# NREL/SSRS

Measured on AMD Instinct MI355X. Metric: simulated tracks/sec (whole node), higher is better.
Workload: dtype f64

## Files before the change

ssrs_amd/csrc/tracks.hip:

```cpp
#include <rocrand/rocrand_philox4x32_10.h>
#include <hipcub/hipcub.hpp>

#include <cmath>
#include <cstdlib>
#include <cstring>
#include <new>
#include <vector>

#include "common.h"
#include "track_plan.h"
#include "track_policy.h"

namespace ssrs {

__host__ __device__ constexpr int dr_of(int k) { return k / 3 - 1; }
__host__ __device__ constexpr int dc_of(int k) { return k % 3 - 1; }
#define SSRS_NINV_DIAG 0.70710677f

constexpr uint32_t restriction(int d)
{
    const int dr = dr_of(d), dc = dc_of(d);
    uint32_t m = 0;
    for (int k = 0; k < 9; ++k) {
        bool ok = false;
// ... 55 lines not shown
    for (int c = 0; c < 8; ++c)
        if (kRingK[c] == k) return c;
    return 8;
}
constexpr bool ring_matches_restrictions()
{
    for (int c = 0; c < 8; ++c) {
        const uint32_t m = (1u << kRingK[(c + 7) % 8]) | (1u << kRingK[c]) | (1u << kRingK[(c + 1) % 8]);
        if (m != restriction(kRingK[c])) return false;
    }
    return true;
}
static_assert(ring_matches_restrictions(), "restriction(d) = ring neighbours of d");
constexpr uint32_t ring_order(int c)
{
    const int ks[3] = {kRingK[(c + 7) % 8], kRingK[c], kRingK[(c + 1) % 8]};
    uint32_t v = 0;
    int n = 0;
    for (int k = 0; k < 9; ++k)
        for (int j = 0; j < 3; ++j)
            if (ks[j] == k) v |= static_cast<uint32_t>(j) << (2 * n++);
    return v;
}
constexpr uint64_t pack_ring_orders()
{
    uint64_t v = 0;
    for (int c = 0; c < 8; ++c) v |= static_cast<uint64_t>(ring_order(c)) << (6 * c);
    return v;
}
constexpr uint64_t kRingOrder = pack_ring_orders();
constexpr uint32_t kOrdId = 0u | (1u << 2) | (2u << 4), kOrdRot = 2u | (0u << 2) | (1u << 4),
                   kOrdRev = 2u | (1u << 2) | (0u << 4), kOrdSwp = 1u | (0u << 2) | (2u << 4);
static_assert(ring_order(0) == kOrdId && ring_order(6) == kOrdId && ring_order(7) == kOrdId, "x0 x1 x2");
static_assert(ring_order(1) == kOrdRot, "after NE: x2 x0 x1");
static_assert(ring_order(2) == kOrdRev && ring_order(3) == kOrdRev && ring_order(4) == kOrdRev, "x2 x1 x0");
static_assert(ring_order(5) == kOrdSwp, "after SW: x1 x0 x2");
static_assert(ring_order(0) == (0u | (1u << 2) | (2u << 4)), "after N: NW, N, NE are k = 6, 7, 8");
static_assert(ring_order(2) == (2u | (1u << 2) | (0u << 4)), "after E: NE, E, SE are k = 8, 5, 2");
constexpr uint32_t pack_ring_deltas(bool rows)
{
    uint32_t v = 1u << 16;
    for (int c = 0; c < 8; ++c)
        v |= static_cast<uint32_t>((rows ? dr_of(kRingK[c]) : dc_of(kRingK[c])) + 1) << (2 * c);
    return v;
}
constexpr uint32_t kRingDr = pack_ring_deltas(true), kRingDc = pack_ring_deltas(false);
constexpr uint32_t pack_ring_next(int sel)
{
    uint32_t v = 0;
    for (int c = 0; c < 8; ++c) v |= static_cast<uint32_t>((c + 7 + ((ring_order(c) >> (2 * sel)) & 3u)) & 7u) << (4 * c);
    return v;
}
constexpr uint32_t kRingNext0 = pack_ring_next(0), kRingNext1 = pack_ring_next(1), kRingNext2 = pack_ring_next(2);
constexpr uint32_t pack_ring_deltas_signed(bool rows)
{
    uint32_t v = 0;
    for (int c = 0; c < 8; ++c)
        v |= (static_cast<uint32_t>(rows ? dr_of(kRingK[c]) : dc_of(kRingK[c])) & 3u) << (4 * c);
    return v;
}
constexpr uint32_t kRingDrS = pack_ring_deltas_signed(true), kRingDcS = pack_ring_deltas_signed(false);
constexpr uint64_t pack_ring_of_k()
{
    uint64_t v = 0;
    for (int k = 0; k < 9; ++k) v |= static_cast<uint64_t>(ring_of_k(k)) << (4 * k);
    return v;
}
constexpr uint64_t kRingOfK = pack_ring_of_k();
constexpr uint64_t pack_k_of_ring()
{
    uint64_t v = 4ull << 32;
    for (int c = 0; c < 8; ++c) v |= static_cast<uint64_t>(kRingK[c]) << (4 * c);
    return v;
}
constexpr uint64_t kKOfRing = pack_k_of_ring();
constexpr int kRingFloats = 10;
__host__ __device__ constexpr size_t ring_mask_offset(int rows, int cols)
{
    return static_cast<size_t>(rows) * static_cast<size_t>(cols) * kRingFloats * sizeof(float) + 8;
}

__device__ __forceinline__ uint4 philox_block(uint64_t seed, uint64_t track, uint64_t blk)
{
#ifdef SSRS_PROBE_NO_PHILOX
    const uint32_t h = static_cast<uint32_t>(blk) * 0x9E3779B9u ^ static_cast<uint32_t>(track) * 0x85EBCA6Bu ^
                       static_cast<uint32_t>(seed);
    return make_uint4(h * 0xC2B2AE35u, h ^ 0x27D4EB2Fu, (h >> 3) * 0x165667B1u, h + 0x9E3779B9u);
#endif
    rocrand_state_philox4x32_10 st;
    rocrand_init(seed, track, blk * 4ull, &st);
    return rocrand4(&st);
}

__device__ __forceinline__ uint4 philox_block_b3(uint64_t seed, uint64_t track, uint64_t blk)
{
    uint32_t c0 = static_cast<uint32_t>(blk), c1 = static_cast<uint32_t>(blk >> 32);
    uint32_t c2 = static_cast<uint32_t>(track), c3 = static_cast<uint32_t>(track >> 32);
    uint32_t k0 = static_cast<uint32_t>(seed), k1 = static_cast<uint32_t>(seed >> 32);
#pragma unroll
    for (int r = 0; r < 10; ++r) {
        const uint64_t p0 = static_cast<uint64_t>(0xD2511F53u) * c0, p1 = static_cast<uint64_t>(0xCD9E8D57u) * c2;
        const uint32_t n0 = __builtin_amdgcn_bitop3_b32(static_cast<uint32_t>(p1 >> 32), c1, k0, 0x96);
        const uint32_t n2 = __builtin_amdgcn_bitop3_b32(static_cast<uint32_t>(p0 >> 32), c3, k1, 0x96);
        c1 = static_cast<uint32_t>(p1);
        c3 = static_cast<uint32_t>(p0);
        c0 = n0;
// ... 1537 lines not shown
    }
    const unsigned long long live = __ballot(active);
    const int lane = threadIdx.x & 63;
    const int nsurv = __popcll(live);
    uint32_t basei = 0;
    if (HM == 6) {
        __shared__ uint32_t s_surv[kBlock / 64 + 1];
        const int wv = threadIdx.x >> 6;
        if (lane == 0) s_surv[wv] = static_cast<uint32_t>(nsurv);
        __syncthreads();
        if (threadIdx.x == 0) {
            uint32_t tot = 0;
            for (int q = 0; q < kBlock / 64; ++q) tot += s_surv[q];
            s_surv[kBlock / 64] = tot ? atomicAdd(&ctl->count[out_slot][xcd], static_cast<uint32_t>(kBlock)) : 0xFFFFFFFFu;
        }
        __syncthreads();
        basei = s_surv[kBlock / 64];
        if (basei != 0xFFFFFFFFu) {
            a.list_out[xcd * a.cap + basei + threadIdx.x] = active ? t : -1;
            if (active) {
                TrackState o;
                o.pos = static_cast<int32_t>(row | (col << 16));
                o.k = k;
                o.dirs = static_cast<uint32_t>(kKOfRing >> (4 * rc)) & 0xFu;
                o.aux = s.aux;
                a.state[t] = o;
            }
        }
    } else {
        if (lane == 0 && nsurv) basei = atomicAdd(&ctl->count[out_slot][xcd], static_cast<uint32_t>(nsurv));
        basei = __shfl(basei, 0);
    }
    if (HM != 6 && active) {
        const int rank = __popcll(live & ((1ull << lane) - 1ull));
        a.list_out[xcd * a.cap + basei + rank] = t;
        TrackState o;
        o.pos = static_cast<int32_t>(row | (col << 16));
        o.k = k;
        o.dirs = static_cast<uint32_t>(kKOfRing >> (4 * rc)) & 0xFu;
        o.aux = s.aux;
        a.state[t] = o;
    }
    unsigned long long mv = live0 ? static_cast<unsigned long long>(k - s.k) : 0ull;
#pragma unroll
    for (int off = 32; off > 0; off >>= 1) mv += __shfl_down(mv, off);
    if (lane == 0 && mv) atomicAdd(&ctl->steps, mv);
}

struct alignas(16) RoamEntry {
    uint32_t e0, ea, eb, ec;
};
static_assert(sizeof(RoamEntry) == 16, "one dwordx4 per state");
constexpr size_t kPairMaxCells = 1ull << 25;

template <bool REV>
__global__ __launch_bounds__(kBlock) void k_roam_build(const char *__restrict__ tab, uint32_t guard, int plane_shift,
                                                      int rows, int cols, RoamEntry *__restrict__ out, const ThrPrior pr)
{
    const uint32_t nstate = static_cast<uint32_t>(rows) * static_cast<uint32_t>(cols) * 8u;
    for (uint32_t s = blockIdx.x * kBlock + threadIdx.x; s < nstate; s += gridDim.x * kBlock) {
        const uint32_t rc = s & 7u, cell = s >> 3;
        auto entry = [&](uint32_t c, uint32_t q) {
            return *reinterpret_cast<const uint32_t *>(tab + (guard + (q << plane_shift)) + (c << 2));
        };
        uint4 en = make_uint4(entry(cell, rc), kThrPoison, kThrPoison, kThrPoison);
        const bool rev = REV && en.x == kThrReversal;
        const uint32_t eu = rev ? pr.rev_e : en.x, rcd = rev ? pr.rev_rc : rc;
        if ((eu & 0xFFFFu) <= (eu >> 16)) {
            const uint32_t ord = static_cast<uint32_t>(kRingOrder >> (6u * rcd)) & 63u;
            uint32_t es[3];
#pragma unroll
            for (int j = 0; j < 3; ++j) {
                const uint32_t ncj = (rcd + 7u + ((ord >> (2 * j)) & 3u)) & 7u;
                const uint32_t cj = cell + ((kRingDr >> (2u * ncj)) & 3u) * static_cast<uint32_t>(cols) + ((kRingDc >> (2u * ncj)) & 3u) -
                                    static_cast<uint32_t>(cols) - 1u;
                es[j] = entry(cj, ncj);
            }
            en.y = es[0]; en.z = es[1]; en.w = es[2];
        }
        reinterpret_cast<uint4 *>(out)[s] = en;
    }
}

struct FineEntry { uint32_t t1, t2; };
struct FinePrior { uint32_t zero_t1[8], zero_t2[8], reversal; };

__host__ __device__ __forceinline__ uint32_t fine_fixed(double x)
{
    const double v = x * 4294967296.0 + 0.5;
    return v >= 4294967295.0 ? 0xFFFFFFFFu : static_cast<uint32_t>(static_cast<unsigned long long>(v));
}

template <bool HAS_POT>
__global__ __launch_bounds__(kBlock) void k_fine_build(const double *__restrict__ updraft, const float *__restrict__ potential,
                                                      FineEntry *__restrict__ out, int rows, int cols, int tiles_x, int ntiles,
                                                      const FinePrior fp)
{
    constexpr int LW = kTabW + 2, LH = kTabH + 2;
    __shared__ double s_inv[LW * LH];
    __shared__ float s_pot[LW * LH];
    const int t = xcd_band(blockIdx.x, ntiles);
    const int r0 = (t / tiles_x) * kTabH, c0 = (t % tiles_x) * kTabW;
    for (int i = threadIdx.x; i < LW * LH; i += kBlock) {
        const int lr = i / LW, lc = i - lr * LW;
        int gr = r0 - 1 + lr, gc = c0 - 1 + lc;
        gr = gr < 0 ? 0 : (gr >= rows ? rows - 1 : gr);
        gc = gc < 0 ? 0 : (gc >= cols ? cols - 1 : gc);
        const size_t g = static_cast<size_t>(gr) * cols + gc;
        const double v = updraft[g];
        const double w = v != v ? v : (v > 1e-06 ? v : 1e-06);
        s_inv[i] = 1.0 / w;
        s_pot[i] = HAS_POT ? potential[g] : 0.f;
    }
    __syncthreads();
    const int lc = static_cast<int>(threadIdx.x % kTabW) + 1;
    const int col = c0 + lc - 1;
    if (col >= cols) return;
    for (int lr = static_cast<int>(threadIdx.x / kTabW) + 1; lr <= kTabH; lr += kBlock / kTabW) {
        const int row = r0 + lr - 1;
        if (row >= rows) break;
        const size_t cell = static_cast<size_t>(row) * cols + col;
        const bool interior = row > 0 && col > 0 && row < rows - 1 && col < cols - 1;
        double w[9];
        bool bad = !interior;
        if (interior) {
            const double ic = s_inv[lr * LW + lc];
            const float pc = s_pot[lr * LW + lc];
#pragma unroll
            for (int j = 0; j < 9; ++j) {
                const int o = (lr + dr_of(j)) * LW + lc + dc_of(j);
                w[j] = 2.0 / (ic + s_inv[o]);
                if (HAS_POT) {
                    const float d = pc - s_pot[o];
                    const float ninv = (j == 4) ? 0.f : ((j & 1) ? 1.f : SSRS_NINV_DIAG);
                    const float e = d * ninv;
                    w[j] = w[j] * static_cast<double>(e);
                }
                bad |= !(w[j] - w[j] == 0.0);
                w[j] = w[j] > 0.0 ? w[j] : 0.0;
            }
        }
        FineEntry en[8];
#pragma unroll
        for (int rc = 0; rc < 8; ++rc) {
            const uint32_t ord = ring_order(rc);
            const int ring3[3] = {(rc + 7) % 8, rc, (rc + 1) % 8};
            const int ka = kRingK[ring3[ord & 3u]], kb = kRingK[ring3[(ord >> 2) & 3u]], kc = kRingK[ring3[(ord >> 4) & 3u]];
            FineEntry e = {0xFFFFFFFFu, 0u};
            if (!bad) {
                const double ab = w[ka] + w[kb], tot = ab + w[kc];
                if (tot == 0.0) {
                    if (!((fp.reversal >> rc) & 1u)) { e.t1 = fp.zero_t1[rc]; e.t2 = fp.zero_t2[rc]; }
                } else if (tot - tot == 0.0) {
                    e.t1 = fine_fixed(w[ka] / tot);
                    e.t2 = fine_fixed(ab / tot);
                    if (e.t1 > e.t2) e.t1 = e.t2;
                }
            }
            en[rc] = e;
        }
        uint4 *dst = reinterpret_cast<uint4 *>(out + cell * 8);
#pragma unroll
        for (int q = 0; q < 4; ++q) dst[q] = make_uint4(en[2 * q].t1, en[2 * q].t2, en[2 * q + 1].t1, en[2 * q + 1].t2);
    }
}

template <bool REV, int BT = kBlock>
__global__ __launch_bounds__(BT) void k_step_roam(const StepArgs a, const ThrPrior pr)
{
    __shared__ uint32_t s_win[kWinRows * kWinCols];
    __shared__ int s_box[4];
    __shared__ int s_wid[BT / 64];
    for (int q = threadIdx.x; q < kWinRows * kWinCols; q += BT) s_win[q] = 0u;
    if (threadIdx.x == 0) { s_box[0] = s_box[1] = 0x7fffffff; s_box[2] = s_box[3] = -1; }
    __syncthreads();
    TrackCtl *ctl = a.ctl;
    const int in_slot = a.launch & 3, out_slot = (a.launch + 1) & 3;
    const uint32_t xcd = blockIdx.x % kXcd;
    const uint32_t nlive = ctl->count[in_slot][xcd];
    const uint32_t il = (blockIdx.x / kXcd) * BT + threadIdx.x;
    const uint32_t i = xcd * a.cap + il;
    if (blockIdx.x == 0 && threadIdx.x < kXcd) ctl->count[(a.launch + 2) & 3][threadIdx.x] = 0;

    bool live0 = il < nlive;
    int32_t t = live0 ? (a.list_in ? a.list_in[i] : static_cast<int32_t>(i)) : 0;
    if (t < 0) { live0 = false; t = 0; }
    TrackState s = {0, -1, 0, 0};
    if (live0) s = a.state[t];
    uint32_t rc = static_cast<uint32_t>(kRingOfK >> (4 * (s.dirs & 0xFu))) & 0xFu;
    live0 = live0 && s.k >= 0 && rc < 8u;
    rc &= 7u;
    int row = s.pos & 0xFFFF, col = (s.pos >> 16) & 0xFFFF;
    int win_r0 = 0, win_c0 = 0;
    {
        int r_lo = live0 ? row : 0x7fffffff, r_hi = live0 ? row : -1, c_lo = live0 ? col : 0x7fffffff, c_hi = live0 ? col : -1;
#pragma unroll
        for (int off = 32; off > 0; off >>= 1) {
            int o = __shfl_xor(r_lo, off); r_lo = o < r_lo ? o : r_lo;
            o = __shfl_xor(r_hi, off); r_hi = o > r_hi ? o : r_hi;
            o = __shfl_xor(c_lo, off); c_lo = o < c_lo ? o : c_lo;
            o = __shfl_xor(c_hi, off); c_hi = o > c_hi ? o : c_hi;
        }
        if ((threadIdx.x & 63) == 0 && r_hi >= 0) {
            atomicMin(&s_box[0], r_lo); atomicMin(&s_box[1], c_lo);
            atomicMax(&s_box[2], r_hi); atomicMax(&s_box[3], c_hi);
        }
        __syncthreads();
        const bool fits = s_box[2] - s_box[0] < kWinRows && s_box[3] - s_box[1] < kWinCols;
        const int nwin = a.wander->n;
        int wid = live0 && nwin > 0 ? wander_window_of(a.wander, nwin, row, col) : 0x7fffffff;
        wid = wid >= nwin ? 0x7fffffff : wid;
        {
            const unsigned long long lm = __ballot(wid != 0x7fffffff);
            wid = lm ? __shfl(wid, __ffsll(static_cast<long long>(lm)) - 1) : 0x7fffffff;
        }
        if ((threadIdx.x & 63) == 0) s_wid[threadIdx.x >> 6] = wid;
        __syncthreads();
        wid = 0x7fffffff;
        for (int q = BT / 64 - 1; q >= 0; --q) wid = s_wid[q] != 0x7fffffff ? s_wid[q] : wid;
        if (wid != 0x7fffffff && threadIdx.x == 0) {
            s_box[0] = a.wander->r0[wid]; s_box[2] = s_box[0] + kWinRows - 1;
            s_box[1] = a.wander->c0[wid]; s_box[3] = s_box[1] + kWinCols - 1;
        }
        const bool placed = wid != 0x7fffffff;
        __syncthreads();
        if (!placed && !fits && threadIdx.x == 0) { s_box[0] = r_lo; s_box[1] = c_lo; s_box[2] = r_hi; s_box[3] = c_hi; }
        __syncthreads();
        if (s_box[2] >= 0) {
            win_r0 = (s_box[0] + s_box[2] + 1 - kWinRows) / 2;
            win_c0 = (s_box[1] + s_box[3] + 1 - kWinCols) / 2;
        }
    }
    const char *pair = reinterpret_cast<const char *>(a.roam);
    const uint32_t ucols = static_cast<uint32_t>(a.cols);
    const uint32_t last_cell = static_cast<uint32_t>(a.rows) * ucols - 1u;
    int k = s.k;
    const long long rel64 = (a.coherent ? static_cast<long long>(s.aux >> 9) : 0) + 1 - a.it_base;
    const int rel = rel64 > 0x3fffffffLL ? 0x3fffffff : (rel64 < 0 ? 0 : static_cast<int>(rel64));
    const long long left = a.max_k - k;
    uint32_t span = !live0 ? 0u : (left > 0x3fffffffLL ? 0x3fffffffu : (left < 0 ? 0u : static_cast<uint32_t>(left)));
    const int blk0 = (k - rel) >> 1;
    const unsigned long long track = a.track_base + static_cast<unsigned long long>(t);
    const char *tab = reinterpret_cast<const char *>(a.table);
    const uint32_t psh = static_cast<uint32_t>(a.plane_shift);
    const uint32_t rev_e = pr.rev_e;
    uint32_t win_stray = 0, n_fine = 0;
    const void *fine = a.fine;

    int wr = 0, wc = 0, lcell = 0;
    bool fast = false;
    uint4 E = make_uint4(kThrPoison, kThrPoison, kThrPoison, kThrPoison);
    auto enter = [&](bool released) __attribute__((always_inline)) {
        wr = row - win_r0;
        wc = col - win_c0;
        lcell = row * a.cols + col;
        fast = live0 && released && span != 0u && k > a.burnin;
        const uint32_t sidx = fast ? ((static_cast<uint32_t>(lcell) << 3) | rc) : 0u;
        E = *reinterpret_cast<const uint4 *>(pair + (sidx << 4));
    };
    enter(rel == 0);
    const uint32_t rev_rc4 = 4u * pr.rev_rc;

    auto slow_step = [&](const uint32_t w0, const uint32_t w1) __attribute__((always_inline)) {
        const uint32_t ufi = w0 >> 16;
        const uint32_t cell = static_cast<uint32_t>(row) * ucols + static_cast<uint32_t>(col);
        const uint32_t e = *reinterpret_cast<const uint32_t *>(tab + (a.guard + (rc << psh)) + (cell << 2));
        const int32_t d1 = static_cast<int32_t>(ufi) - static_cast<int32_t>(e & 0xFFFFu);
        const int32_t d2 = static_cast<int32_t>(ufi) - static_cast<int32_t>(e >> 16);
        const bool burn = k <= a.burnin;
        bool special = (static_cast<uint32_t>(d1 + 1) < 2u) | (static_cast<uint32_t>(d2 + 1) < 2u) | (d1 < d2);
        if (burn) special |= (row <= 1) | (row >= a.rows - 2) | (col >= a.cols - 2);
        uint32_t nc;
        int br = row, bc = col;
        if (!special) {
            const uint32_t ord = static_cast<uint32_t>(kRingOrder >> (6u * rc)) & 63u;
            const uint32_t neg = (static_cast<uint32_t>(d1) >> 31) + (static_cast<uint32_t>(d2) >> 31);
            nc = (rc + 7u + ((ord >> (4u - 2u * neg)) & 3u)) & 7u;
        } else {
            if (e == kThrBoundary && !burn) { span = 0u; return; }
            bool exact = true;
            nc = 0;
            if (fine && !(d1 < d2) && !(burn && ((row <= 1) | (row >= a.rows - 2) | (col >= a.cols - 2)))) {
                const uint2 f = reinterpret_cast<const uint2 *>(fine)[(cell << 3) | rc];
                const uint32_t u32 = (w0 & ~31u) | (w1 >> 27);
                const long long f1 = static_cast<long long>(u32) - static_cast<long long>(f.x);
                const long long f2 = static_cast<long long>(u32) - static_cast<long long>(f.y);
                const bool unsure = (f.x > f.y) | (static_cast<unsigned long long>(f1 + 1) < 2ull) | (static_cast<unsigned long long>(f2 + 1) < 2ull);
                if (!unsure) {
                    const uint32_t ord = static_cast<uint32_t>(kRingOrder >> (6u * rc)) & 63u;
                    const uint32_t neg = (f1 < 0 ? 1u : 0u) + (f2 < 0 ? 1u : 0u);
                    nc = (rc + 7u + ((ord >> (4u - 2u * neg)) & 3u)) & 7u;
                    exact = false;
                    ++n_fine;
                }
            }
            if (e == kThrReversal && !burn) {
                int idx = 0;
                bool near = false;
#pragma unroll
                for (int q = 0; q < 9; ++q) {
                    const int32_t d = static_cast<int32_t>(ufi) - static_cast<int32_t>(pr.thr9[q]);
                    idx += d >= 0 ? 1 : 0;
                    near |= static_cast<uint32_t>(d + 1) < 2u;
                }
                const uint32_t pnc = static_cast<uint32_t>(kRingOfK >> (4 * (idx > 8 ? 4 : idx))) & 0xFu;
                if (!near && pnc < 8u) { nc = pnc; exact = false; }
            }
            if (exact) {
                int er = row, ec = col;
                if (burn) {
                    if (er <= 1) er += 2; else if (er >= a.rows - 2) er -= 2;
                    if (ec <= 0) ec += 2; else if (ec >= a.cols - 2) ec -= 2;
                }
                double w[9];
                if (a.potential) window_weights<true>(a.updraft, a.potential, a.cols, er, ec, w);
                else window_weights<false>(a.updraft, a.potential, a.cols, er, ec, w);
                double prr[9];
#pragma unroll
                for (int j = 0; j < 9; ++j) prr[j] = a.prior[j];
                const uint32_t last = static_cast<uint32_t>(kKOfRing >> (4 * rc)) & 0xFu;
                const int idx = choose_move(w, prr, 1.0, restriction_of(last), words_to_uniform(w0, w1), true);
                nc = static_cast<uint32_t>(kRingOfK >> (4 * idx)) & 0xFu;
                br = er; bc = ec;
            }
        }
        row = br + static_cast<int>((kRingDr >> (2u * nc)) & 3u) - 1;
        col = bc + static_cast<int>((kRingDc >> (2u * nc)) & 3u) - 1;
        rc = nc;
        ++k;
        const uint32_t hr = static_cast<uint32_t>(row - win_r0), hc = static_cast<uint32_t>(col - win_c0);
        if (hr < static_cast<uint32_t>(kWinRows) && hc < static_cast<uint32_t>(kWinCols)) {
            atomicAdd(&s_win[hr * kWinCols + hc], 1u);
        } else {
            atomicAdd(&a.hist[static_cast<uint32_t>(row) * ucols + static_cast<uint32_t>(col)], 1u);
            ++win_stray;
        }
    };

    int it = 0;
    uint32_t n_pairs = 0, n_slow = 0;
    const unsigned long long t_begin = a.debug_roam ? __builtin_amdgcn_s_memtime() : 0ull;
    auto one_pair = [&]() __attribute__((always_inline)) {
        const uint4 w4 = philox_block_b3(a.seed, track, static_cast<unsigned long long>(static_cast<uint32_t>(blk0 + (it >> 1))));
        const uint32_t ufa = w4.x >> 16, ufb = w4.z >> 16;
        const bool st_a = static_cast<uint32_t>(it - rel) < span, st_b = static_cast<uint32_t>(it + 1 - rel) < span;
        const uint32_t q0 = E.x, qa = E.y, qb = E.z, qc = E.w;
        const uint32_t rc0 = rc;
        const uint32_t rc04 = 4u * rc0;
        const bool rva = REV && q0 == kThrReversal;
        const uint32_t eua = rva ? rev_e : q0;
        const uint32_t t4a = rva ? rev_rc4 : rc04;
        const bool ga1 = ufa >= (eua & 0xFFFFu), ga2 = ufa >= (eua >> 16);
        const uint32_t nxa = ga2 ? kRingNext2 : (ga1 ? kRingNext1 : kRingNext0);
        const uint32_t nca = (nxa >> t4a) & 7u, nca4 = 4u * nca;
        const uint32_t q1 = ga2 ? qc : (ga1 ? qb : qa);
        const int dra = __builtin_amdgcn_sbfe(static_cast<int>(kRingDrS), nca4, 2u), dca = __builtin_amdgcn_sbfe(static_cast<int>(kRingDcS), nca4, 2u);
        const int cell_a = lcell + __mul24(dra, a.cols) + dca;
        const bool rvb = REV && q1 == kThrReversal;
        const uint32_t eub = rvb ? rev_e : q1;
        const uint32_t t4b = rvb ? rev_rc4 : nca4;
        const bool gb1 = ufb >= (eub & 0xFFFFu), gb2 = ufb >= (eub >> 16);
        const uint32_t nxb = gb2 ? kRingNext2 : (gb1 ? kRingNext1 : kRingNext0);
        const uint32_t ncb = (nxb >> t4b) & 7u, ncb4 = 4u * ncb;
        const int drb = __builtin_amdgcn_sbfe(static_cast<int>(kRingDrS), ncb4, 2u), dcb = __builtin_amdgcn_sbfe(static_cast<int>(kRingDcS), ncb4, 2u);
        const int cell_b = cell_a + __mul24(drb, a.cols) + dcb;
        {
            const uint32_t cb = static_cast<uint32_t>(cell_b) < last_cell ? static_cast<uint32_t>(cell_b) : last_cell;
            E = *reinterpret_cast<const uint4 *>(pair + ((cb << 7) | (ncb4 << 2)));
        }
        const int wra = wr + dra, wca = wc + dca, wrb = wra + drb, wcb = wca + dcb;
        const int32_t a1 = static_cast<int32_t>(ufa) - static_cast<int32_t>(eua & 0xFFFFu);
        const int32_t a2 = static_cast<int32_t>(ufa) - static_cast<int32_t>(eua >> 16);
        const int32_t b1 = static_cast<int32_t>(ufb) - static_cast<int32_t>(eub & 0xFFFFu);
        const int32_t b2 = static_cast<int32_t>(ufb) - static_cast<int32_t>(eub >> 16);
        const bool special = (static_cast<uint32_t>(a1 + 1) < 2u) | (static_cast<uint32_t>(a2 + 1) < 2u) | (a1 < a2) |
                             (static_cast<uint32_t>(b1 + 1) < 2u) | (static_cast<uint32_t>(b2 + 1) < 2u) | (b1 < b2);
        const bool go = fast & st_a & st_b & !special;
        const bool in_a = go & (static_cast<uint32_t>(wra) < static_cast<uint32_t>(kWinRows)) & (static_cast<uint32_t>(wca) < static_cast<uint32_t>(kWinCols));
        const bool in_b = go & (static_cast<uint32_t>(wrb) < static_cast<uint32_t>(kWinRows)) & (static_cast<uint32_t>(wcb) < static_cast<uint32_t>(kWinCols));
        const bool out = go & !(in_a & in_b);
        const bool slow = (st_a | st_b) & !go;
        const unsigned long long rare = __ballot(out | slow);
        atomicAdd(&s_win[in_a ? (wra << 8) + wca : 0], in_a ? 1u : 0u);
        atomicAdd(&s_win[in_b ? (wrb << 8) + wcb : 0], in_b ? 1u : 0u);
        k += go ? 2 : 0;
        wr = go ? wrb : wr;
        wc = go ? wcb : wc;
        lcell = go ? cell_b : lcell;
        rc = go ? ncb : rc0;
        ++n_pairs;
        if (__builtin_expect(rare != 0ull, 0)) {
            if (__any(out)) {
#ifdef SSRS_PROBE_NO_STRAY_ATOMICS
                if (go && !in_a) ++win_stray;
                if (go && !in_b) ++win_stray;
#else
                if (go && !in_a) { atomicAdd(&a.hist[cell_a], 1u); ++win_stray; }
                if (go && !in_b) { atomicAdd(&a.hist[cell_b], 1u); ++win_stray; }
#endif
            }
            if (__any(slow)) {
                ++n_slow;
                if (slow) {
                    if (fast) { row = win_r0 + wr; col = win_c0 + wc; }
#pragma unroll 1
                    for (int h = 0; h < 2; ++h)
                        if (static_cast<uint32_t>(it + h - rel) < span) slow_step(h ? w4.z : w4.x, h ? w4.w : w4.y);
                    enter(true);
                }
            }
        }
        it += 2;
    };
    const uint32_t stop_stamp = static_cast<uint32_t>(a.launch) + 1u;
    uint32_t stop_seen = 0u;
    bool stopped = false;
    for (; it + 8 <= a.steps; ) {
        const unsigned long long stepping = __ballot(static_cast<uint32_t>(it - rel) < span), waiting = __ballot(it < rel && span != 0u);
        const bool stop_now = a.roam_stop && waiting == 0ull &&
                              static_cast<uint32_t>(__builtin_amdgcn_readfirstlane(static_cast<int>(stop_seen))) == stop_stamp;
        if (((stepping | waiting) == 0ull) | stop_now) { stopped = stop_now; break; }
        if (a.roam_stop) stop_seen = __hip_atomic_load(&ctl->roam_stop, __ATOMIC_RELAXED, __HIP_MEMORY_SCOPE_AGENT);
#pragma unroll
        for (int u = 0; u < 4; ++u) one_pair();
    }
    for (; it < a.steps && !stopped; ) {
        if (!__any(static_cast<uint32_t>(it - rel) < span || (it < rel && span != 0u))) break;
        one_pair();
    }
    if (a.roam_stop && !stopped && it >= a.steps && (threadIdx.x & 63) == 0) atomicMax(&ctl->roam_stop, stop_stamp);
    if (fast) { row = win_r0 + wr; col = win_c0 + wc; }
    {
        uint32_t nf = n_fine;
#pragma unroll
        for (int off = 32; off > 0; off >>= 1) nf += __shfl_down(nf, off);
        if ((threadIdx.x & 63) == 0 && nf) atomicAdd(&ctl->pad, nf);
    }
    if ((threadIdx.x & 63) == 0 && n_pairs) {
        atomicAdd(&ctl->roam_pairs, static_cast<unsigned long long>(n_pairs));
        if (n_slow) atomicAdd(&ctl->roam_slow, static_cast<unsigned long long>(n_slow));
        if (a.debug_roam) {
            const unsigned long long dt = __builtin_amdgcn_s_memtime() - t_begin;
            atomicAdd(&ctl->dbg_tsum, dt);
            atomicMax(&ctl->dbg_tmax, dt);
            atomicAdd(&ctl->dbg_waves, 1ull);
            atomicMax(&ctl->dbg_slowmax, (static_cast<unsigned long long>(n_slow) << 32) | n_pairs);
        }
    }
#ifdef SSRS_DEBUG_WAVE_DUMP
    if (a.debug_roam && a.launch == SSRS_DEBUG_WAVE_DUMP && a.dbg_buf) {
        const unsigned long long dt = __builtin_amdgcn_s_memtime() - t_begin;
        const int lanes = __popcll(__ballot(live0));
        uint32_t wst = win_stray;
        for (int off = 32; off > 0; off >>= 1) wst += __shfl_down(wst, off);
        if ((threadIdx.x & 63) == 0) {
            unsigned long long *r = a.dbg_buf + 8ull * (blockIdx.x * (BT / 64) + (threadIdx.x >> 6));
            r[0] = dt; r[1] = static_cast<unsigned long long>(lanes); r[2] = n_pairs; r[3] = n_slow; r[4] = wst;
            r[5] = static_cast<unsigned long long>(win_r0); r[6] = static_cast<unsigned long long>(win_c0);
            r[7] = static_cast<uint32_t>(__popcll(__ballot(fast)));
        }
    }
#endif
    __syncthreads();
    for (int q = threadIdx.x; q < kWinRows * kWinCols; q += BT) {
        const uint32_t n = s_win[q];
        if (n) atomicAdd(&a.hist[static_cast<uint32_t>(win_r0 + q / kWinCols) * ucols + static_cast<uint32_t>(win_c0 + q % kWinCols)], n);
    }
    {
        unsigned long long ws = win_stray;
#pragma unroll
        for (int off = 32; off > 0; off >>= 1) ws += __shfl_down(ws, off);
        if ((threadIdx.x & 63) == 0 && ws) atomicAdd(&ctl->strays, ws);
    }
    const bool active = live0 && span != 0u && k < static_cast<int>(a.max_k);
    if (live0 && !active) {
        if (a.lengths) a.lengths[t] = static_cast<int32_t>(k + 1);
        if (a.end_rc) reinterpret_cast<uint32_t *>(a.end_rc)[t] = (static_cast<uint32_t>(row) & 0xFFFFu) | (static_cast<uint32_t>(col) << 16);
    }
    __shared__ uint32_t s_surv[BT / 64 + 1];
    const int lane = threadIdx.x & 63, wv = threadIdx.x >> 6;
    const int nsurv = __popcll(__ballot(active));
    if (lane == 0) s_surv[wv] = static_cast<uint32_t>(nsurv);
    __syncthreads();
    if (threadIdx.x == 0) {
// ... 819 lines not shown
#else
    return 0;
#endif
}

static void fine_prior_tables(const double *prior, FinePrior *out)
{
    *out = FinePrior{};
    for (int rc = 0; rc < 8; ++rc) {
        const uint32_t mask = restriction(kRingK[rc]);
        double q[9], qq[9], cdf[9];
        bool any = false;
        for (int k = 0; k < 9; ++k) {
            q[k] = ((mask >> k) & 1u) && k != 4 ? prior[k] : 0.0;
            any |= q[k] != 0.0;
        }
        if (!any) { out->reversal |= 1u << rc; continue; }
        const double s1 = sum9(q);
        for (int k = 0; k < 9; ++k) qq[k] = q[k] / s1;
        const double s2 = sum9(qq);
        double acc = 0.0;
        for (int k = 0; k < 9; ++k) { qq[k] = qq[k] / s2; acc = acc + qq[k]; cdf[k] = acc; }
        const uint32_t ord = ring_order(rc);
        const int ring3[3] = {(rc + 7) % 8, rc, (rc + 1) % 8};
        const int ka = kRingK[ring3[ord & 3u]], kb = kRingK[ring3[(ord >> 2) & 3u]];
        out->zero_t1[rc] = fine_fixed(cdf[ka] / cdf[8]);
        out->zero_t2[rc] = fine_fixed(cdf[kb] / cdf[8]);
        if (out->zero_t1[rc] > out->zero_t2[rc]) out->zero_t1[rc] = out->zero_t2[rc];
    }
}

extern "C" int ssrs_track_params_init(SsrsTrackParams *p, int rows, int cols,
                                      int memory_parameter, double scaling_parameter)
{
    SSRS_REQUIRE(p != nullptr, "ssrs_track_params_init: params is NULL");
    SSRS_REQUIRE(rows >= 5 && cols >= 5, "ssrs_track_params_init: need rows, cols >= 5");
    *p = SsrsTrackParams{};
    p->rows = rows;
    p->cols = cols;
    p->burnin = static_cast<int32_t>((rows < cols ? rows : cols) / 10.0);
    const double mm = rows / 2.0 * cols / 2.0;
    p->max_moves = static_cast<int64_t>(ceil(mm));
    p->memory_parameter = memory_parameter;
    p->scaling_parameter = scaling_parameter;
    return SSRS_OK;
}

extern "C" size_t ssrs_tracks_workspace_bytes(int64_t ntracks)
{
    if (ntracks < 0) ntracks = 0;
    return workspace_layout(ntracks, nullptr, nullptr);
}

static size_t pair_table_bytes(int64_t ntracks, int rows, int cols)
{
    if (ntracks < kWanderMinTracks || rows <= 0 || cols <= 0) return 0;
    const size_t cells = static_cast<size_t>(rows) * static_cast<size_t>(cols);
    return cells < kPairMaxCells ? align_up(cells * 8 * sizeof(RoamEntry), 256) + align_up(cells * 8 * sizeof(FineEntry), 256) : 0;
}

extern "C" size_t ssrs_tracks_workspace_bytes_ex(int64_t ntracks, int rows, int cols, int hist_copies)
{
    const size_t base = align_up(ssrs_tracks_workspace_bytes(ntracks), 256) + pair_table_bytes(ntracks, rows, cols);
    if (rows <= 0 || cols <= 0 || hist_copies < 2) return base;
    if (hist_copies > 64) hist_copies = 64;
    return base + static_cast<size_t>(hist_copies) * static_cast<size_t>(rows) * static_cast<size_t>(cols) * sizeof(uint32_t);
}

extern "C" int ssrs_transition_table_build(const double *updraft, const float *potential,
                                           double *table, int rows, int cols, void *stream)
{
    SSRS_REQUIRE(updraft && table, "ssrs_transition_table_build: updraft/table is NULL");
    SSRS_REQUIRE(rows >= 3 && cols >= 3, "ssrs_transition_table_build: need rows, cols >= 3");
    SSRS_REQUIRE((reinterpret_cast<uintptr_t>(table) & 63u) == 0,
                 "ssrs_transition_table_build: table must be 64-byte aligned");
    const int tx = (cols + kTabW - 1) / kTabW, ty = (rows + kTabH - 1) / kTabH, nt = tx * ty;
    hipLaunchKernelGGL(k_transition_table<false>, dim3(static_cast<unsigned>(nt)), dim3(kBlock), 0,
                       as_stream(stream), updraft, potential, static_cast<void *>(table), rows, cols, tx, nt);
    SSRS_HIP_CHECK(hipGetLastError());
    return SSRS_OK;
}

extern "C" size_t ssrs_transition_ring_bytes(int rows, int cols)
{
    if (rows <= 0 || cols <= 0) return 0;
    const size_t cells = static_cast<size_t>(rows) * static_cast<size_t>(cols);
    return ring_mask_offset(rows, cols) + (cells + 3) / 4 * 4;
}

extern "C" int ssrs_transition_ring_build(const double *updraft, const float *potential,
                                          float *ring, int rows, int cols, void *stream)
{
    SSRS_REQUIRE(updraft && ring, "ssrs_transition_ring_build: updraft/ring is NULL");
    SSRS_REQUIRE(rows >= 3 && cols >= 3, "ssrs_transition_ring_build: need rows, cols >= 3");
    SSRS_REQUIRE((reinterpret_cast<uintptr_t>(ring) & 7u) == 0,
                 "ssrs_transition_ring_build: ring must be 8-byte aligned");
    const int tx = (cols + kTabW - 1) / kTabW, ty = (rows + kTabH - 1) / kTabH, nt = tx * ty;
    hipLaunchKernelGGL(k_transition_table<true>, dim3(static_cast<unsigned>(nt)), dim3(kBlock), 0,
                       as_stream(stream), updraft, potential, static_cast<void *>(ring), rows, cols, tx, nt);
    SSRS_HIP_CHECK(hipGetLastError());
    return SSRS_OK;
}

static size_t thr_guard_bytes(int cols) { return align_up((static_cast<size_t>(cols) + 2) * 4, 256); }

extern "C" size_t ssrs_transition_thr_bytes(int rows, int cols)
{
    if (rows <= 0 || cols <= 0) return 0;
    return (static_cast<size_t>(8) << thr_plane_shift(rows, cols)) + 2 * thr_guard_bytes(cols);
}

// ... 275 lines not shown
        a.dbg_buf = dump_buf;
    }
#endif
    a.cheap_exact = sw.cheap_exact ? 1 : 0;
    a.vcap = ws.cap;
    lean = p->memory_parameter == 1 && c.traj == nullptr;
    ring = (p->flags & SSRS_TRACKS_RING_TABLE) != 0;
    thr = (p->flags & SSRS_TRACKS_THR_TABLE) != 0;
    if (thr) {
        SSRS_REQUIRE(!ring && c.table && c.updraft && lean && a.fast && (S & 1) == 0,
                     "ssrs_tracks_simulate: SSRS_TRACKS_THR_TABLE needs table + updraft, memory_parameter 1, "
                     "scaling_parameter 1, no direct trajectory output, no EXACT_ONLY and an even steps_per_launch");
        SSRS_REQUIRE(static_cast<size_t>(p->rows) * static_cast<size_t>(p->cols) <= (1ull << 26),
                     "ssrs_tracks_simulate: the threshold table needs rows * cols <= 2^26");
        prior_tables(p->prior, &thr_prior);
        a.plane_shift = thr_plane_shift(p->rows, p->cols);
        a.guard = static_cast<uint32_t>(thr_guard_bytes(p->cols));
        a.pf_dir = coherent ? (geom.cos_t > 0.98 ? 1 : (geom.cos_t < -0.98 ? -1 : 0)) : 0;
        a.pf_rc = a.pf_dir < 0 ? 4 : 0;
    }
    if (ring)
        SSRS_REQUIRE(c.table && c.updraft && lean && a.fast && (S & 1) == 0,
                     "ssrs_tracks_simulate: SSRS_TRACKS_RING_TABLE needs table + updraft, memory_parameter 1, "
                     "scaling_parameter 1, no trajectory output, no EXACT_ONLY and an even steps_per_launch");
    return SSRS_OK;
}

int TrackRun::choose_front_path()
{
    const int64_t ntracks = c.ntracks;
    uint32_t *const hist = c.hist;
    const double off_axis = std::fabs(geom.sin_t) < std::fabs(geom.cos_t) ? std::fabs(geom.sin_t) : std::fabs(geom.cos_t);
    ntc = static_cast<uint32_t>((p->cols + kTileCols - 1) / kTileCols);
    ntiles = ntc * static_cast<uint32_t>((p->rows + kTileRows - 1) / kTileRows);
    const bool tiles_ok = hist != nullptr && coherent && S <= kVisitSteps && ntracks >= 8192 && ntiles <= kTilesMax &&
                          static_cast<unsigned long long>(ws.cap) * kXcd * static_cast<unsigned long long>(S) < (1ull << 32) &&
                          (p->flags & SSRS_TRACKS_NO_BINNING) == 0;
    bool tiles_on = tiles_ok && off_axis > 0.17;
    const bool want_transposed = coherent && !tiles_on && std::fabs(geom.sin_t) > std::fabs(geom.cos_t);
    const bool binning = hist != nullptr && coherent && S <= kVisitSteps &&
                         (p->flags & SSRS_TRACKS_NO_BINNING) == 0 &&
                         (want_transposed ? p->rows : p->cols) <= kBinCells;
    a.visits = nullptr;
    a.visit_stride = ws.visit_stride;
    bool binning_on = binning && ntracks >= 8192 && !tiles_on;
    const bool never_scattered = (p->flags & SSRS_TRACKS_NO_SCATTERED) != 0;
    const bool scattered = (p->flags & SSRS_TRACKS_SCATTERED) != 0;
    if (scattered) binning_on = tiles_on = false;
    const bool cache_ok = thr && hist != nullptr && !(c.rec && c.rec->complete) && sw.block_window;
    size_t ws_base = align_up(ssrs_tracks_workspace_bytes(ntracks), 256);
    {
        const size_t pb = thr ? pair_table_bytes(ntracks, p->rows, p->cols) : 0;
        if (pb && c.workspace_bytes >= ws_base + pb) {
            ws.roam = reinterpret_cast<RoamEntry *>(static_cast<char *>(c.workspace) + ws_base);
            if (sw.fine_table)
                a.fine = static_cast<char *>(c.workspace) + ws_base +
                         align_up(static_cast<size_t>(p->rows) * static_cast<size_t>(p->cols) * 8 * sizeof(RoamEntry), 256);
            ws_base += pb;
        }
        a.roam = ws.roam;
    }
    roam_ok = cache_ok && ws.roam != nullptr && sw.roam_table;
    rev = thr_prior.rev_ok != 0 && sw.rev;
    wander_sort_ok = ntracks >= kWanderMinTracks &&
                     static_cast<long long>((p->rows + kBinRows - 1) / kBinRows) * ((p->cols + kBinCols - 1) / kBinCols) <= kWanderBins;
    ncell = static_cast<size_t>(p->rows) * static_cast<size_t>(p->cols);
    if (hist && c.workspace_bytes > ws_base) ncopies = static_cast<int>((c.workspace_bytes - ws_base) / (ncell * sizeof(uint32_t)));
    uint32_t *extra = reinterpret_cast<uint32_t *>(static_cast<char *>(c.workspace) + ws_base);
    if (want_transposed && binning_on) {
        if (ncopies >= 1) { hist_t = extra; extra += ncell; --ncopies; }
        else binning_on = false;
    }
    if (hist_t) SSRS_HIP_CHECK(hipMemsetAsync(hist_t, 0, sizeof(uint32_t) * ncell, st));
    ncopies = ncopies > 64 ? 64 : ncopies;
    copies_ptr = ncopies >= 2 ? extra : nullptr;
    a.hist_copies = nullptr;
    a.ncopies = 1;
    a.zmask = ring ? reinterpret_cast<const uint8_t *>(c.table) + ring_mask_offset(p->rows, p->cols) : nullptr;
    v16_ok = 5ll * p->cols <= kBinCells;
    a.v16_offset = geom.offset;

    pol.thr = thr; pol.tiles_ok = tiles_ok; pol.cache_ok = cache_ok; pol.never_scattered = never_scattered;
    pol.front = a.pf_dir != 0; pol.may_rebalance = sw.rebalance; pol.debug = sw.debug; pol.roam_shuffle = sw.roam_shuffle;
    pol.ntracks = ntracks; pol.crossing = p->rows + p->cols;
    pol.binning_on = binning_on; pol.tiles_on = tiles_on; pol.scattered = scattered;
    pol.cached = cache_ok && scattered;
    pol.want_wander_sort = pol.cached;
    pol.upper = static_cast<uint32_t>(ntracks < static_cast<int64_t>(ws.cap) ? ntracks : ws.cap);
    ev.own_batch = !profile;
    if (!profile)
        for (int i = 0; i < kRing; ++i) SSRS_HIP_CHECK(hipEventCreate(&ev.batch[i]));
    return SSRS_OK;
}

int TrackRun::launch_steps(bool first_move, unsigned blocks, uint32_t *vcap, long long *vstride) const
{
    *vcap = ws.cap;
    *vstride = ws.visit_stride;
    if (first_move) return 1;
    const bool recording = c.rec && c.rec->complete;
    if (thr && pol.cached && !recording && sw.grow_steps) {
        return (roam_ok && roam_ready && pol.stable_roam >= 2) ? 128 * S : 8 * S;
    }
    if (thr && (pol.binning_on || pol.tiles_on) && !recording && sw.grow_steps) {
        const uint32_t vc = (blocks / kXcd) * kBlock;
        const long long room = (ws.visit_stride * kVisitSteps) / (static_cast<long long>(kXcd) * vc);
        long long grown = room < 8ll * S ? room : 8ll * S;
        grown &= ~1ll;
        if (grown >= S + S / 4) {
            *vcap = vc;
// ... 545 lines not shown
```

Baseline: 75260.

## Pad roam pair table with poison bands and shorten inner-loop address math

Adds poisoned guard bands of two rows before and after the roam pair table, so the inner step loop can index neighbour cells without clamping to the last cell. Cell indices are kept pre-scaled (shifted by 7) and ring indices pre-multiplied by 4, and the next-ring lookup uses rotated constants with alignbit. Scheduling barriers and DPP lane copies are also added to shape instruction scheduling. The cost is a slightly larger workspace and a more fragile layout: the guard bands must exactly cover every out-of-range access, and the workspace size calculation changes with them.

```diff
diff --git a/ssrs_amd/csrc/tracks.hip b/ssrs_amd/csrc/tracks.hip
--- a/ssrs_amd/csrc/tracks.hip
+++ b/ssrs_amd/csrc/tracks.hip
@@ -131,6 +131,18 @@
     return v;
 }
 constexpr uint32_t kRingNext0 = pack_ring_next(0), kRingNext1 = pack_ring_next(1), kRingNext2 = pack_ring_next(2);
+constexpr uint32_t rotl2(uint32_t v) { return (v << 2) | (v >> 30); }
+constexpr uint32_t kRingNextR0 = rotl2(kRingNext0), kRingNextR1 = rotl2(kRingNext1), kRingNextR2 = rotl2(kRingNext2);
+constexpr bool ring_next_rotated_ok(uint32_t plain, uint32_t rotated)
+{
+    for (uint32_t c = 0; c < 8; ++c) {
+        const uint32_t r = c ? (rotated >> (4 * c)) | (rotated << (32 - 4 * c)) : rotated;
+        if ((r & 28u) != 4u * ((plain >> (4 * c)) & 7u)) return false;
+    }
+    return true;
+}
+static_assert(ring_next_rotated_ok(kRingNext0, kRingNextR0) && ring_next_rotated_ok(kRingNext1, kRingNextR1) &&
+              ring_next_rotated_ok(kRingNext2, kRingNextR2), "rotated next-ring constants decode like the plain ones");
 constexpr uint32_t pack_ring_deltas_signed(bool rows)
 {
     uint32_t v = 0;
@@ -1774,13 +1786,21 @@
 };
 static_assert(sizeof(RoamEntry) == 16, "one dwordx4 per state");
 constexpr size_t kPairMaxCells = 1ull << 25;
+__host__ __device__ constexpr uint32_t pair_band_cells(int cols) { return 2u * (static_cast<uint32_t>(cols) + 1u); }
 
 template <bool REV>
 __global__ __launch_bounds__(kBlock) void k_roam_build(const char *__restrict__ tab, uint32_t guard, int plane_shift,
                                                       int rows, int cols, RoamEntry *__restrict__ out, const ThrPrior pr)
 {
     const uint32_t nstate = static_cast<uint32_t>(rows) * static_cast<uint32_t>(cols) * 8u;
-    for (uint32_t s = blockIdx.x * kBlock + threadIdx.x; s < nstate; s += gridDim.x * kBlock) {
+    const uint32_t nband = pair_band_cells(cols) * 8u;
+    uint4 *const out_b = reinterpret_cast<uint4 *>(out) - nband;
+    for (uint32_t sb = blockIdx.x * kBlock + threadIdx.x; sb < nstate + 2u * nband; sb += gridDim.x * kBlock) {
+        const uint32_t s = sb - nband;
+        if (s >= nstate) {
+            out_b[sb] = make_uint4(kThrPoison, kThrPoison, kThrPoison, kThrPoison);
+            continue;
+        }
         const uint32_t rc = s & 7u, cell = s >> 3;
         auto entry = [&](uint32_t c, uint32_t q) {
             return *reinterpret_cast<const uint32_t *>(tab + (guard + (q << plane_shift)) + (c << 2));
@@ -1800,7 +1820,7 @@
             }
             en.y = es[0]; en.z = es[1]; en.w = es[2];
         }
-        reinterpret_cast<uint4 *>(out)[s] = en;
+        out_b[sb] = en;
     }
 }
 
@@ -1887,6 +1907,11 @@
     }
 }
 
+__device__ __forceinline__ uint32_t lane_copy(uint32_t v)
+{
+    return static_cast<uint32_t>(__builtin_amdgcn_mov_dpp(static_cast<int>(v), 0xE4, 0xF, 0xF, true));
+}
+
 template <bool REV, int BT = kBlock>
 __global__ __launch_bounds__(BT) void k_step_roam(const StepArgs a, const ThrPrior pr)
 {
@@ -1953,9 +1978,10 @@
             win_c0 = (s_box[1] + s_box[3] + 1 - kWinCols) / 2;
         }
     }
-    const char *pair = reinterpret_cast<const char *>(a.roam);
     const uint32_t ucols = static_cast<uint32_t>(a.cols);
-    const uint32_t last_cell = static_cast<uint32_t>(a.rows) * ucols - 1u;
+    const uint32_t band = pair_band_cells(a.cols);
+    const char *pair = reinterpret_cast<const char *>(a.roam) - (static_cast<size_t>(band) << 7);
+    const int cols7 = a.cols << 7;
     int k = s.k;
     const long long rel64 = (a.coherent ? static_cast<long long>(s.aux >> 9) : 0) + 1 - a.it_base;
     const int rel = rel64 > 0x3fffffffLL ? 0x3fffffff : (rel64 < 0 ? 0 : static_cast<int>(rel64));
@@ -1965,23 +1991,23 @@
     const unsigned long long track = a.track_base + static_cast<unsigned long long>(t);
     const char *tab = reinterpret_cast<const char *>(a.table);
     const uint32_t psh = static_cast<uint32_t>(a.plane_shift);
-    const uint32_t rev_e = pr.rev_e;
+    const uint32_t rev_e = lane_copy(pr.rev_e), rev_rc4 = lane_copy(4u * pr.rev_rc);
     uint32_t win_stray = 0, n_fine = 0;
     const void *fine = a.fine;
 
-    int wr = 0, wc = 0, lcell = 0;
+    int wr = 0, wc = 0;
+    uint32_t lc7 = 0, rc4 = 0;
     bool fast = false;
     uint4 E = make_uint4(kThrPoison, kThrPoison, kThrPoison, kThrPoison);
     auto enter = [&](bool released) __attribute__((always_inline)) {
         wr = row - win_r0;
         wc = col - win_c0;
-        lcell = row * a.cols + col;
+        lc7 = (static_cast<uint32_t>(row * a.cols + col) + band) << 7;
+        rc4 = 4u * rc;
         fast = live0 && released && span != 0u && k > a.burnin;
-        const uint32_t sidx = fast ? ((static_cast<uint32_t>(lcell) << 3) | rc) : 0u;
-        E = *reinterpret_cast<const uint4 *>(pair + (sidx << 4));
+        E = *reinterpret_cast<const uint4 *>(pair + (fast ? (lc7 | (rc4 << 2)) : (band << 7)));
     };
     enter(rel == 0);
-    const uint32_t rev_rc4 = 4u * pr.rev_rc;
 
     auto slow_step = [&](const uint32_t w0, const uint32_t w1) __attribute__((always_inline)) {
         const uint32_t ufi = w0 >> 16;
@@ -2066,30 +2092,27 @@
         const uint4 w4 = philox_block_b3(a.seed, track, static_cast<unsigned long long>(static_cast<uint32_t>(blk0 + (it >> 1))));
         const uint32_t ufa = w4.x >> 16, ufb = w4.z >> 16;
         const bool st_a = static_cast<uint32_t>(it - rel) < span, st_b = static_cast<uint32_t>(it + 1 - rel) < span;
+        const uint32_t rc04 = rc4;
+        __builtin_amdgcn_sched_barrier(0);
         const uint32_t q0 = E.x, qa = E.y, qb = E.z, qc = E.w;
-        const uint32_t rc0 = rc;
-        const uint32_t rc04 = 4u * rc0;
         const bool rva = REV && q0 == kThrReversal;
         const uint32_t eua = rva ? rev_e : q0;
         const uint32_t t4a = rva ? rev_rc4 : rc04;
         const bool ga1 = ufa >= (eua & 0xFFFFu), ga2 = ufa >= (eua >> 16);
-        const uint32_t nxa = ga2 ? kRingNext2 : (ga1 ? kRingNext1 : kRingNext0);
-        const uint32_t nca = (nxa >> t4a) & 7u, nca4 = 4u * nca;
+        const uint32_t nxa = ga2 ? kRingNextR2 : (ga1 ? kRingNextR1 : kRingNextR0);
+        const uint32_t nca4 = __builtin_amdgcn_alignbit(nxa, nxa, t4a) & 28u;
         const uint32_t q1 = ga2 ? qc : (ga1 ? qb : qa);
         const int dra = __builtin_amdgcn_sbfe(static_cast<int>(kRingDrS), nca4, 2u), dca = __builtin_amdgcn_sbfe(static_cast<int>(kRingDcS), nca4, 2u);
-        const int cell_a = lcell + __mul24(dra, a.cols) + dca;
         const bool rvb = REV && q1 == kThrReversal;
         const uint32_t eub = rvb ? rev_e : q1;
         const uint32_t t4b = rvb ? rev_rc4 : nca4;
         const bool gb1 = ufb >= (eub & 0xFFFFu), gb2 = ufb >= (eub >> 16);
-        const uint32_t nxb = gb2 ? kRingNext2 : (gb1 ? kRingNext1 : kRingNext0);
-        const uint32_t ncb = (nxb >> t4b) & 7u, ncb4 = 4u * ncb;
+        const uint32_t nxb = gb2 ? kRingNextR2 : (gb1 ? kRingNextR1 : kRingNextR0);
+        const uint32_t ncb4 = __builtin_amdgcn_alignbit(nxb, nxb, t4b) & 28u;
         const int drb = __builtin_amdgcn_sbfe(static_cast<int>(kRingDrS), ncb4, 2u), dcb = __builtin_amdgcn_sbfe(static_cast<int>(kRingDcS), ncb4, 2u);
-        const int cell_b = cell_a + __mul24(drb, a.cols) + dcb;
-        {
-            const uint32_t cb = static_cast<uint32_t>(cell_b) < last_cell ? static_cast<uint32_t>(cell_b) : last_cell;
-            E = *reinterpret_cast<const uint4 *>(pair + ((cb << 7) | (ncb4 << 2)));
-        }
+        const uint32_t cell_b7 = lc7 + static_cast<uint32_t>(__mul24(dra + drb, cols7)) + (static_cast<uint32_t>(dca + dcb) << 7);
+        E = *reinterpret_cast<const uint4 *>(pair + (cell_b7 | (ncb4 << 2)));
+        __builtin_amdgcn_sched_barrier(0);
         const int wra = wr + dra, wca = wc + dca, wrb = wra + drb, wcb = wca + dcb;
         const int32_t a1 = static_cast<int32_t>(ufa) - static_cast<int32_t>(eua & 0xFFFFu);
         const int32_t a2 = static_cast<int32_t>(ufa) - static_cast<int32_t>(eua >> 16);
@@ -2108,8 +2131,8 @@
         k += go ? 2 : 0;
         wr = go ? wrb : wr;
         wc = go ? wcb : wc;
-        lcell = go ? cell_b : lcell;
-        rc = go ? ncb : rc0;
+        lc7 = go ? cell_b7 : lc7;
+        rc4 = go ? ncb4 : rc04;
         ++n_pairs;
         if (__builtin_expect(rare != 0ull, 0)) {
             if (__any(out)) {
@@ -2117,14 +2140,16 @@
                 if (go && !in_a) ++win_stray;
                 if (go && !in_b) ++win_stray;
 #else
-                if (go && !in_a) { atomicAdd(&a.hist[cell_a], 1u); ++win_stray; }
-                if (go && !in_b) { atomicAdd(&a.hist[cell_b], 1u); ++win_stray; }
+                const uint32_t cell_a7 = cell_b7 - static_cast<uint32_t>(__mul24(drb, cols7)) - (static_cast<uint32_t>(dcb) << 7);
+                if (go && !in_a) { atomicAdd(&a.hist[(cell_a7 >> 7) - band], 1u); ++win_stray; }
+                if (go && !in_b) { atomicAdd(&a.hist[(cell_b7 >> 7) - band], 1u); ++win_stray; }
 #endif
             }
             if (__any(slow)) {
                 ++n_slow;
                 if (slow) {
                     if (fast) { row = win_r0 + wr; col = win_c0 + wc; }
+                    rc = rc4 >> 2;
 #pragma unroll 1
                     for (int h = 0; h < 2; ++h)
                         if (static_cast<uint32_t>(it + h - rel) < span) slow_step(h ? w4.z : w4.x, h ? w4.w : w4.y);
@@ -2152,6 +2177,7 @@
     }
     if (a.roam_stop && !stopped && it >= a.steps && (threadIdx.x & 63) == 0) atomicMax(&ctl->roam_stop, stop_stamp);
     if (fast) { row = win_r0 + wr; col = win_c0 + wc; }
+    rc = rc4 >> 2;
     {
         uint32_t nf = n_fine;
 #pragma unroll
@@ -3077,11 +3103,17 @@
     return workspace_layout(ntracks, nullptr, nullptr);
 }
 
+static size_t pair_front_band_bytes(int cols) { return static_cast<size_t>(pair_band_cells(cols)) * 8 * sizeof(RoamEntry); }
+static size_t pair_banded_bytes(int rows, int cols)
+{
+    return align_up((static_cast<size_t>(rows) * static_cast<size_t>(cols) + 2 * static_cast<size_t>(pair_band_cells(cols))) * 8 * sizeof(RoamEntry), 256);
+}
 static size_t pair_table_bytes(int64_t ntracks, int rows, int cols)
 {
     if (ntracks < kWanderMinTracks || rows <= 0 || cols <= 0) return 0;
     const size_t cells = static_cast<size_t>(rows) * static_cast<size_t>(cols);
-    return cells < kPairMaxCells ? align_up(cells * 8 * sizeof(RoamEntry), 256) + align_up(cells * 8 * sizeof(FineEntry), 256) : 0;
+    return cells + 2 * static_cast<size_t>(pair_band_cells(cols)) < kPairMaxCells
+               ? pair_banded_bytes(rows, cols) + align_up(cells * 8 * sizeof(FineEntry), 256) : 0;
 }
 
 extern "C" size_t ssrs_tracks_workspace_bytes_ex(int64_t ntracks, int rows, int cols, int hist_copies)
@@ -3463,10 +3495,8 @@
     {
         const size_t pb = thr ? pair_table_bytes(ntracks, p->rows, p->cols) : 0;
         if (pb && c.workspace_bytes >= ws_base + pb) {
-            ws.roam = reinterpret_cast<RoamEntry *>(static_cast<char *>(c.workspace) + ws_base);
-            if (sw.fine_table)
-                a.fine = static_cast<char *>(c.workspace) + ws_base +
-                         align_up(static_cast<size_t>(p->rows) * static_cast<size_t>(p->cols) * 8 * sizeof(RoamEntry), 256);
+            ws.roam = reinterpret_cast<RoamEntry *>(static_cast<char *>(c.workspace) + ws_base + pair_front_band_bytes(p->cols));
+            if (sw.fine_table) a.fine = static_cast<char *>(c.workspace) + ws_base + pair_banded_bytes(p->rows, p->cols);
             ws_base += pb;
         }
         a.roam = ws.roam;
```

Result: no change. 74930 (-0.4%).
